# microsoft/ORBIT-Dataset

Hardware: AMD Instinct MI355X
Metric: query frames/sec per task (224×224, 5-way ProtoNet) + frame accuracy vs ref (higher is better)
Workload: dtype f32

## Files before the change

include/orbit_hip.h:

```cpp
#ifndef ORBIT_HIP_H
#define ORBIT_HIP_H

#include <stddef.h>
#include <stdint.h>

#ifdef __cplusplus
extern "C" {
#endif

typedef struct orbit_extractor orbit_extractor_t;
typedef struct orbit_filmgen orbit_filmgen_t;
typedef struct orbit_vit orbit_vit_t;
typedef void* orbit_stream_t;

#define ORBIT_OK 0
#define ORBIT_ERR_ARG (-1)
#define ORBIT_ERR_HIP (-2)
#define ORBIT_ERR_STATE (-3)
#define ORBIT_ERR_NOMEM (-4)

#define ORBIT_ACT_NONE 0
#define ORBIT_ACT_RELU 1
#define ORBIT_ACT_SILU 2
#define ORBIT_ACT_ELU 3
// ... 22 lines not shown
                        int n_tasks, int M, int T, int D, int C, float logit_scale, int cosine,
                        float* logits, int32_t* argmax, orbit_stream_t stream);

int orbit_mean_pool(const float* x, int N, int T, int D, float* out, orbit_stream_t stream);

int orbit_history_mean_pool(const float* x, int F, int T, int D, float* out, orbit_stream_t stream);
int orbit_set_mean(const float* x, int n, int D, float* out, orbit_stream_t stream);

int orbit_extractor_create(const char* name, int H, int W, orbit_extractor_t** out);
#define ORBIT_PLAN_UNFUSED 1
int orbit_extractor_create_ex(const char* name, int H, int W, int flags, orbit_extractor_t** out);
void orbit_extractor_destroy(orbit_extractor_t* fe);

int orbit_extractor_num_params(const orbit_extractor_t* fe);
const char* orbit_extractor_param_name(const orbit_extractor_t* fe, int i);
size_t orbit_extractor_param_numel(const orbit_extractor_t* fe, int i);

int orbit_extractor_load(orbit_extractor_t* fe, const char* key, const float* data, size_t numel);
int orbit_extractor_load_async(orbit_extractor_t* fe, const char* key, const float* device_data, size_t numel,
                               orbit_stream_t stream);
int orbit_extractor_load_all_async(orbit_extractor_t* fe, const float* const* device_ptrs, int n, orbit_stream_t stream);
int orbit_extractor_finalize(orbit_extractor_t* fe, orbit_stream_t stream);

int orbit_extractor_output_size(const orbit_extractor_t* fe);
int orbit_extractor_film_slots(const orbit_extractor_t* fe);
int orbit_extractor_film_slot_channels(const orbit_extractor_t* fe, int slot);
const char* orbit_extractor_film_slot_name(const orbit_extractor_t* fe, int slot);
int orbit_extractor_film_size(const orbit_extractor_t* fe);

size_t orbit_extractor_workspace_bytes(const orbit_extractor_t* fe, int B);
double orbit_extractor_macs_per_frame(const orbit_extractor_t* fe);

int orbit_extractor_forward(orbit_extractor_t* fe, const float* frames, int B,
                            const float* film_gamma, const float* film_beta,
                            float* feats, void* workspace, size_t workspace_bytes, orbit_stream_t stream);

int orbit_vit_create(const char* name, int H, int W, orbit_vit_t** out);
void orbit_vit_destroy(orbit_vit_t* v);
int orbit_vit_num_params(const orbit_vit_t* v);
const char* orbit_vit_param_name(const orbit_vit_t* v, int i);
size_t orbit_vit_param_numel(const orbit_vit_t* v, int i);
int orbit_vit_load(orbit_vit_t* v, const char* key, const float* data, size_t numel);
int orbit_vit_load_async(orbit_vit_t* v, const char* key, const float* device_data, size_t numel, orbit_stream_t stream);
int orbit_vit_load_all_async(orbit_vit_t* v, const float* const* device_ptrs, int n, orbit_stream_t stream);
int orbit_vit_finalize(orbit_vit_t* v, orbit_stream_t stream);
int orbit_vit_output_size(const orbit_vit_t* v);
int orbit_vit_film_slots(const orbit_vit_t* v);
int orbit_vit_film_slot_channels(const orbit_vit_t* v, int slot);
const char* orbit_vit_film_slot_name(const orbit_vit_t* v, int slot);
int orbit_vit_film_size(const orbit_vit_t* v);
size_t orbit_vit_workspace_bytes(const orbit_vit_t* v, int B);
double orbit_vit_macs_per_frame(const orbit_vit_t* v);
int orbit_vit_forward(orbit_vit_t* v, const float* frames, int B, const float* film_gamma, const float* film_beta,
                      float* feats, void* workspace, size_t workspace_bytes, orbit_stream_t stream);
size_t orbit_vit_tape_bytes(const orbit_vit_t* v, int B);
size_t orbit_vit_backward_workspace_bytes(const orbit_vit_t* v, int B);
int orbit_vit_train_forward(orbit_vit_t* v, const float* frames, int B, const float* film_gamma, const float* film_beta,
                            float* feats, void* tape, size_t tape_bytes, void* workspace, size_t workspace_bytes,
                            orbit_stream_t stream);
int orbit_vit_backward(orbit_vit_t* v, int B, const float* film_gamma, const float* film_beta, const float* dfeats,
                       const void* tape, size_t tape_bytes, float* dgamma, float* dbeta, void* workspace,
                       size_t workspace_bytes, orbit_stream_t stream);

int orbit_filmgen_create(int n_gen, int z_dim, int hidden, const int* out_size, const int* kind,
                         const int* dst_offset, orbit_filmgen_t** out);
void orbit_filmgen_destroy(orbit_filmgen_t* g);
int orbit_filmgen_load(orbit_filmgen_t* g, int gen, const char* tensor, const float* data, size_t numel);
int orbit_filmgen_load_all_async(orbit_filmgen_t* g, const float* const* device_ptrs, int n, orbit_stream_t stream);
int orbit_filmgen_forward(orbit_filmgen_t* g, const float* z, float* film_gamma, float* film_beta,
                          float* l2, orbit_stream_t stream);

int orbit_op_conv2d(const float* x, int x_nchw, const float* w, float* y,
                    const float* scale, const float* shift, const float* residual, const float* gate,
                    int B, int H, int W, int Cin, int Cout, int KH, int KW, int stride,
                    int pad_top, int pad_left, int Ho, int Wo, int act, int pool2,
                    orbit_stream_t stream);
int orbit_op_pw_stream(const float* x, const float* w, const float* scale, const float* shift, const float* residual,
                       const float* partial, int chunks, const float* w1, const float* b1, const float* w2t, const float* b2,
                       int R, float* y, float* gate_out, int B, int H, int W, int Cin, int Cout, orbit_stream_t stream);
int orbit_pw_stream_supported(int Cin, int Cout, int H, int W);
int orbit_op_dwconv2d(const float* x, const float* w, float* y, const float* scale, const float* shift,
                      int B, int H, int W, int C, int K, int stride, int pad_top, int pad_left,
                      int Ho, int Wo, int act, orbit_stream_t stream);
int orbit_op_conv2d_train(const float* x, int x_nchw, const float* w, float* y, const float* gate, int B, int H, int W,
                          int Cin, int Cout, int KH, int KW, int stride, int pad_top, int pad_left, int Ho, int Wo,
                          float* stats, int* stat_blocks, orbit_stream_t stream);
int orbit_op_dwconv2d_train(const float* x, const float* w, float* y, const float* in_scale, const float* in_shift,
                            int in_act, int B, int H, int W, int C, int K, int stride, int pad_top, int pad_left, int Ho,
                            int Wo, float* stats, orbit_stream_t stream);
int orbit_op_maxpool2d(const float* x, float* y, int B, int H, int W, int C, int K, int stride, int pad,
                       int Ho, int Wo, orbit_stream_t stream);
int orbit_op_avgpool(const float* x, float* y, int B, int HW, int C, orbit_stream_t stream);
int orbit_op_se_gate(const float* pooled, const float* w1, const float* b1, const float* w2,
                     const float* b2, float* gate, int B, int C, int R, orbit_stream_t stream);

int orbit_op_vit_linear(const float* x, const float* w, const float* bias, const float* residual, float* y, int M, int N,
                        int K, int epilogue, int tile_rows, orbit_stream_t stream);
int orbit_op_vit_patch_embed(const float* frames, const float* w, const float* bias_or_null, const float* pos_embed,
                             const float* cls_token, float* tokens, int B, int D, int tile_rows, orbit_stream_t stream);
int orbit_op_vit_layernorm(const float* x, size_t x_stride, float* y, size_t y_stride, int rows, int D, const float* gamma,
                           const float* beta, float eps, orbit_stream_t stream);
int orbit_op_vit_attention(const float* qkv, float* out, int B, int D, int heads, orbit_stream_t stream);
int orbit_op_vit_linear_dgrad(const float* dy, const float* w, float* wt_scratch, const float* u, const float* residual,
                              float* dx, int M, int N, int K, int tile_rows, orbit_stream_t stream);
int orbit_op_vit_layernorm_bwd(const float* x, size_t x_stride, const float* dy, size_t dy_stride, const float* gamma, float eps,
                               const float* dres, float* dx, size_t dx_stride, int rows, int D, float* dgamma, float* dbeta,
                               float* partial, size_t partial_floats, orbit_stream_t stream);
int orbit_op_vit_attention_bwd(const float* qkv, const float* dout, float* dqkv, int B, int D, int heads,
                               orbit_stream_t stream);

int orbit_op_mbconv_front_partials(int H, int W, int Cin, int mid, int K, int stride);
int orbit_op_mbconv_front(const float* x, const float* w1, const float* scale1, const float* shift1,
                          const float* wdw, const float* scale2, const float* shift2, float* y, float* pool_partial,
                          int B, int H, int W, int Cin, int mid, int K, int stride, int pad_top, int pad_left,
                          int Ho, int Wo, orbit_stream_t stream);
int orbit_op_stem_dw_front_partials(int H, int W, int mid);
int orbit_op_stem_dw_front(const float* frames, const float* w_stem, const float* scale1, const float* shift1,
                           const float* wdw, const float* scale2, const float* shift2, float* y, float* pool_partial,
                           int B, int FH, int FW, int spad_top, int spad_left, int H, int W, int mid, int pad_top,
                           int pad_left, int Ho, int Wo, orbit_stream_t stream);

int orbit_dense_rows(const float* x, int R, int in, const float* W, const float* b, int out, int act,
                     const float* residual, float* y, orbit_stream_t stream);
int orbit_spd_inverse(const float* A, float* Ainv, int n, int batch, orbit_stream_t stream);
size_t orbit_mahalanobis_workspace_bytes(int N, int M, int D, int C);
int orbit_mahalanobis_configure(const float* features, const int64_t* labels, const int64_t* class_ids, int N, int D,
                                int C, float* means, float* task_mean, float* precisions, float* task_precision,
                                void* workspace, size_t workspace_bytes, orbit_stream_t stream);
int orbit_mahalanobis_predict(const float* features, const float* means, const float* precisions, int M, int D, int C,
                              float logit_scale, float* logits, void* workspace, size_t workspace_bytes,
                              orbit_stream_t stream);

int orbit_mahalanobis_predict_backward(const float* dlogits, const float* features, const float* means,
                                       const float* precisions, int M, int D, int C, float logit_scale, float* dfeatures,
                                       void* workspace, size_t workspace_bytes, orbit_stream_t stream);

int orbit_extractor_supports_training(const orbit_extractor_t* fe);
size_t orbit_extractor_tape_bytes(const orbit_extractor_t* fe, int B);
size_t orbit_extractor_backward_workspace_bytes(const orbit_extractor_t* fe, int B);
size_t orbit_extractor_grad_floats(const orbit_extractor_t* fe);
size_t orbit_extractor_param_offset(const orbit_extractor_t* fe, int i);
size_t orbit_extractor_bn_stat_floats(const orbit_extractor_t* fe);
int orbit_extractor_export_bn_stats(orbit_extractor_t* fe, float* dst, orbit_stream_t stream);
int orbit_extractor_train_forward(orbit_extractor_t* fe, const float* frames, int B, const float* film_gamma,
                                  const float* film_beta, int bn_train, float momentum, float* feats, void* tape,
                                  size_t tape_bytes, orbit_stream_t stream);
#define ORBIT_TRAIN_NO_BACKWARD 1
#define ORBIT_TRAIN_DEFER_RUNNING_STATS 2
int orbit_extractor_train_forward_ex(orbit_extractor_t* fe, const float* frames, int B, const float* film_gamma,
                                     const float* film_beta, int bn_train, float momentum, float* feats, void* tape,
                                     size_t tape_bytes, int flags, orbit_stream_t stream);
int orbit_extractor_apply_deferred_bn_stats(orbit_extractor_t* fe, const void* tape, size_t tape_bytes, int B, float momentum,
                                            orbit_stream_t stream);
int orbit_extractor_backward(orbit_extractor_t* fe, const float* frames, int B, const float* film_gamma,
                             const float* film_beta, int bn_train, const float* dfeats, const void* tape,
                             size_t tape_bytes, float* param_grads, int filter_grads, float* dfilm_gamma,
                             float* dfilm_beta, void* workspace, size_t workspace_bytes, orbit_stream_t stream);
int orbit_extractor_train_graph_stats(const orbit_extractor_t* fe, long* replays, long* eager);
size_t orbit_filmgen_grad_floats(const orbit_filmgen_t* g);
size_t orbit_filmgen_param_offset(const orbit_filmgen_t* g, int gen, const char* tensor);
int orbit_filmgen_backward(orbit_filmgen_t* g, const float* z, const float* dfilm_gamma, const float* dfilm_beta,
                           const float* dl2, float* grads, float* dz, orbit_stream_t stream);
int orbit_proto_predict_backward(const float* dlogits, const float* features, const float* weight, int M, int T, int D,
                                 int C, float logit_scale, int cosine, float* dfeatures, orbit_stream_t stream);

int orbit_linear_head_backward(const float* dlogits, const float* features, int M, int D, int C, float logit_scale,
// ... 77 lines not shown
```

orbit-dataset_amd/_lib.py:

```python
import ctypes
import os
from ctypes import c_char_p, c_double, c_float, c_int, c_size_t, c_void_p, POINTER

_HERE = os.path.dirname(os.path.abspath(__file__))
LIB_PATH = os.path.join(_HERE, "lib", "liborbit_hip.so")

_lib = None

P = c_void_p
_SIGNATURES = {
    "orbit_version": (c_int, []),
    "orbit_last_error": (c_char_p, []),
    "orbit_device_count": (c_int, []),
    "orbit_set_option": (c_int, [c_char_p, c_int]),
    "orbit_get_option": (c_int, [c_char_p]),
    "orbit_label_set": (c_int, [P, c_int, P, c_int, P, P]),
    "orbit_proto_configure": (c_int, [P, P, P, c_int, c_int, c_int, c_int, c_int, P, P, P]),
    "orbit_proto_finalize": (c_int, [P, P, c_int, c_int, c_int, c_int, P, P, P]),
    "orbit_proto_predict": (c_int, [P, P, P, c_int, c_int, c_int, c_int, c_int, c_float, c_int, P, P, P]),
    "orbit_mean_pool": (c_int, [P, c_int, c_int, c_int, P, P]),
    "orbit_set_mean": (c_int, [P, c_int, c_int, P, P]),
    "orbit_history_mean_pool": (c_int, [P, c_int, c_int, c_int, P, P]),
    "orbit_extractor_create": (c_int, [c_char_p, c_int, c_int, POINTER(c_void_p)]),
    "orbit_extractor_create_ex": (c_int, [c_char_p, c_int, c_int, c_int, POINTER(c_void_p)]),
    "orbit_extractor_destroy": (None, [P]),
    "orbit_extractor_num_params": (c_int, [P]),
    "orbit_extractor_param_name": (c_char_p, [P, c_int]),
    "orbit_extractor_param_numel": (c_size_t, [P, c_int]),
    "orbit_extractor_load": (c_int, [P, c_char_p, P, c_size_t]),
    "orbit_extractor_load_async": (c_int, [P, c_char_p, P, c_size_t, P]),
    "orbit_extractor_load_all_async": (c_int, [P, P, c_int, P]),
    "orbit_extractor_finalize": (c_int, [P, P]),
    "orbit_extractor_output_size": (c_int, [P]),
    "orbit_extractor_film_slots": (c_int, [P]),
    "orbit_extractor_film_slot_channels": (c_int, [P, c_int]),
    "orbit_extractor_film_slot_name": (c_char_p, [P, c_int]),
    "orbit_extractor_film_size": (c_int, [P]),
    "orbit_extractor_workspace_bytes": (c_size_t, [P, c_int]),
    "orbit_extractor_macs_per_frame": (c_double, [P]),
    "orbit_extractor_forward": (c_int, [P, P, c_int, P, P, P, P, c_size_t, P]),
    "orbit_vit_create": (c_int, [c_char_p, c_int, c_int, POINTER(c_void_p)]),
    "orbit_vit_destroy": (None, [P]),
    "orbit_vit_num_params": (c_int, [P]),
    "orbit_vit_param_name": (c_char_p, [P, c_int]),
    "orbit_vit_param_numel": (c_size_t, [P, c_int]),
    "orbit_vit_load": (c_int, [P, c_char_p, P, c_size_t]),
    "orbit_vit_load_async": (c_int, [P, c_char_p, P, c_size_t, P]),
    "orbit_vit_load_all_async": (c_int, [P, P, c_int, P]),
    "orbit_vit_finalize": (c_int, [P, P]),
    "orbit_vit_output_size": (c_int, [P]),
    "orbit_vit_film_slots": (c_int, [P]),
    "orbit_vit_film_slot_channels": (c_int, [P, c_int]),
    "orbit_vit_film_slot_name": (c_char_p, [P, c_int]),
    "orbit_vit_film_size": (c_int, [P]),
    "orbit_vit_workspace_bytes": (c_size_t, [P, c_int]),
    "orbit_vit_macs_per_frame": (c_double, [P]),
    "orbit_vit_forward": (c_int, [P, P, c_int, P, P, P, P, c_size_t, P]),
    "orbit_vit_tape_bytes": (c_size_t, [P, c_int]),
    "orbit_vit_backward_workspace_bytes": (c_size_t, [P, c_int]),
    "orbit_vit_train_forward": (c_int, [P, P, c_int, P, P, P, P, c_size_t, P, c_size_t, P]),
    "orbit_vit_backward": (c_int, [P, c_int, P, P, P, P, c_size_t, P, P, P, c_size_t, P]),
    "orbit_filmgen_create": (c_int, [c_int, c_int, c_int, POINTER(c_int), POINTER(c_int), POINTER(c_int),
                                     POINTER(c_void_p)]),
    "orbit_filmgen_destroy": (None, [P]),
    "orbit_filmgen_load": (c_int, [P, c_int, c_char_p, P, c_size_t]),
    "orbit_filmgen_load_all_async": (c_int, [P, P, c_int, P]),
    "orbit_filmgen_forward": (c_int, [P, P, P, P, P, P]),
    "orbit_op_conv2d": (c_int, [P, c_int, P, P, P, P, P, P] + [c_int] * 14 + [P]),
    "orbit_op_dwconv2d": (c_int, [P, P, P, P, P] + [c_int] * 11 + [P]),
    "orbit_op_pw_stream": (c_int, [P] * 6 + [c_int] + [P] * 4 + [c_int, P, P] + [c_int] * 5 + [P]),
    "orbit_pw_stream_supported": (c_int, [c_int] * 4),
    "orbit_op_conv2d_train": (c_int, [P, c_int, P, P, P] + [c_int] * 12 + [P, POINTER(c_int), P]),
    "orbit_op_dwconv2d_train": (c_int, [P, P, P, P, P] + [c_int] * 11 + [P, P]),
    "orbit_op_maxpool2d": (c_int, [P, P] + [c_int] * 9 + [P]),
    "orbit_op_avgpool": (c_int, [P, P, c_int, c_int, c_int, P]),
    "orbit_op_se_gate": (c_int, [P, P, P, P, P, P, c_int, c_int, c_int, P]),
    "orbit_op_vit_linear": (c_int, [P] * 5 + [c_int] * 5 + [P]),
    "orbit_op_vit_patch_embed": (c_int, [P] * 6 + [c_int] * 3 + [P]),
    "orbit_op_vit_layernorm": (c_int, [P, c_size_t, P, c_size_t, c_int, c_int, P, P, c_float, P]),
    "orbit_op_vit_attention": (c_int, [P, P, c_int, c_int, c_int, P]),
    "orbit_op_vit_linear_dgrad": (c_int, [P] * 6 + [c_int] * 4 + [P]),
    "orbit_op_vit_layernorm_bwd": (c_int, [P, c_size_t, P, c_size_t, P, c_float, P, P, c_size_t, c_int, c_int, P, P, P,
                                           c_size_t, P]),
    "orbit_op_vit_attention_bwd": (c_int, [P, P, P, c_int, c_int, c_int, P]),
    "orbit_op_mbconv_front": (c_int, [P] * 9 + [c_int] * 11 + [P]),
    "orbit_op_mbconv_front_partials": (c_int, [c_int] * 6),
    "orbit_op_stem_dw_front_partials": (c_int, [c_int] * 3),
    "orbit_op_stem_dw_front": (c_int, [P] * 9 + [c_int] * 12 + [P]),
    "orbit_dense_rows": (c_int, [P, c_int, c_int, P, P, c_int, c_int, P, P, P]),
    "orbit_spd_inverse": (c_int, [P, P, c_int, c_int, P]),
    "orbit_mahalanobis_workspace_bytes": (c_size_t, [c_int, c_int, c_int, c_int]),
    "orbit_mahalanobis_configure": (c_int, [P, P, P, c_int, c_int, c_int, P, P, P, P, P, c_size_t, P]),
    "orbit_mahalanobis_predict": (c_int, [P, P, P, c_int, c_int, c_int, c_float, P, P, c_size_t, P]),
    "orbit_mahalanobis_predict_backward": (c_int, [P, P, P, P, c_int, c_int, c_int, c_float, P, P, c_size_t, P]),
    "orbit_extractor_supports_training": (c_int, [P]),
    "orbit_extractor_tape_bytes": (c_size_t, [P, c_int]),
    "orbit_extractor_backward_workspace_bytes": (c_size_t, [P, c_int]),
    "orbit_extractor_grad_floats": (c_size_t, [P]),
    "orbit_extractor_param_offset": (c_size_t, [P, c_int]),
    "orbit_extractor_bn_stat_floats": (c_size_t, [P]),
    "orbit_extractor_export_bn_stats": (c_int, [P, P, P]),
    "orbit_extractor_train_forward": (c_int, [P, P, c_int, P, P, c_int, c_float, P, P, c_size_t, P]),
    "orbit_extractor_train_forward_ex": (c_int, [P, P, c_int, P, P, c_int, c_float, P, P, c_size_t, c_int, P]),
    "orbit_extractor_apply_deferred_bn_stats": (c_int, [P, P, c_size_t, c_int, c_float, P]),
    "orbit_extractor_backward": (c_int, [P, P, c_int, P, P, c_int, P, P, c_size_t, P, c_int, P, P, P, c_size_t, P]),
    "orbit_filmgen_grad_floats": (c_size_t, [P]),
    "orbit_filmgen_param_offset": (c_size_t, [P, c_int, c_char_p]),
    "orbit_filmgen_backward": (c_int, [P, P, P, P, P, P, P, P]),
    "orbit_proto_predict_backward": (c_int, [P, P, P, c_int, c_int, c_int, c_int, c_float, c_int, P, P]),
    "orbit_linear_head_backward": (c_int, [P, P, c_int, c_int, c_int, c_float, P, P, P]),
    "orbit_cross_entropy_forward": (c_int, [P, P, c_int, c_int, c_int, P, P, P, P]),
    "orbit_cross_entropy_backward": (c_int, [P, P, P, c_int, c_int, c_int, P, P]),
    "orbit_op_bn_train_forward": (c_int, [P, c_int, c_int, P, P, c_float, c_float, P, P, P, c_int, P, P, P, P]),
    "orbit_op_bn_stats_from_gram": (c_int, [P, c_int, c_int, P, c_int, c_float, P, P, P]),
    "orbit_op_bn_backward": (c_int, [P, P, P, c_int, c_int, P, P, P, c_int, c_int, P, P, P, P, P]),
    "orbit_op_conv2d_dgrad": (c_int, [P, P, P, P] + [c_int] * 12 + [P]),
    "orbit_op_conv2d_wgrad": (c_int, [P, c_int, P, P] + [c_int] * 12 + [P]),
    "orbit_op_conv2d_wgrad_gated": (c_int, [P, P, P, P] + [c_int] * 5 + [P]),
    "orbit_op_maxpool2d_train": (c_int, [P, P, P] + [c_int] * 9 + [P]),
    "orbit_op_maxpool2d_backward": (c_int, [P, P, P] + [c_int] * 9 + [P]),
    "orbit_op_avgpool_backward": (c_int, [P, P, c_int, c_int, c_int, P]),
    "orbit_op_dwconv2d_backward": (c_int, [P, P, P, P, P] + [c_int] * 10 + [P]),
    "orbit_op_dwconv2d_dgrad_bn": (c_int, [P] * 7 + [c_int, P, P, P] + [c_int] * 10 + [P]),
    "orbit_op_dwconv2d_wgrad_xf": (c_int, [P, P, P, c_int, P, P] + [c_int] * 10 + [P]),
    "orbit_op_se_gate_backward": (c_int, [P] * 12 + [c_int] * 4 + [P]),
    "orbit_frames_from_uint8": (c_int, [P, c_int, c_int, c_int, c_int, POINTER(c_float), POINTER(c_float), P, P]),
    "orbit_prof_enable": (c_int, [c_int]),
    "orbit_prof_collect": (c_int, [POINTER(c_double), POINTER(c_double), POINTER(ctypes.c_long)]),
    "orbit_prof_num_variants": (c_int, []),
    "orbit_prof_variant": (c_int, [c_int, ctypes.c_char_p, POINTER(ctypes.c_long), POINTER(c_double),
                                   POINTER(c_double), POINTER(c_double)]),
    "orbit_prof_set_roofs": (c_int, [c_double, c_double, c_double]),
    "orbit_prof_variant_floor": (c_int, [c_int, POINTER(c_double), POINTER(c_double), POINTER(c_double)]),
    "orbit_runtime_init": (c_int, []),
    "orbit_comm_unique_id": (c_int, [P]),
    "orbit_comm_init": (c_int, [c_int, c_int, P]),
    "orbit_comm_world": (c_int, []),
    "orbit_comm_rank": (c_int, []),
    "orbit_allreduce_sum": (c_int, [P, c_size_t, P]),
    "orbit_extractor_train_graph_stats": (c_int, [P, P, P]),
    "orbit_comm_destroy": (None, []),
    "orbit_p2p_create": (c_int, [c_int, c_int, c_size_t, POINTER(c_void_p)]),
    "orbit_p2p_export": (c_int, [P, P]),
    "orbit_p2p_connect": (c_int, [P, P]),
    "orbit_p2p_allreduce_sum": (c_int, [P, P, c_size_t, P]),
    "orbit_p2p_allreduce_sum_sharded": (c_int, [P, P, c_size_t, P]),
    "orbit_p2p_error": (c_int, [P]),
    "orbit_p2p_memory_kind": (c_int, [P]),
    "orbit_p2p_destroy": (None, [P]),
}

EXPORTS = tuple(_SIGNATURES)
# ... 120 lines not shown
```

orbit-dataset_amd/csrc/ops.hip:

```cpp
#include "common.h"
#include "device_util.h"
#include "se_gate.h"
#include <algorithm>

namespace orbit {

using v4f = __attribute__((ext_vector_type(4))) float;

struct DwInXf {
    const float* scale;
    const float* shift;
    int act;
};
struct DwBnbVec {
    v4f sc, sh, mu, is;
};
__device__ __forceinline__ v4f dw_bnb(v4f dx, v4f yv, const DwBnbVec& b, int act, v4f& s0, v4f& s1) {
    const v4f z = yv * b.sc + b.sh;
    v4f g = dx;
    if (act == ORBIT_ACT_SILU) {
#pragma unroll
        for (int k = 0; k < 4; ++k) {
            const float sg = __builtin_amdgcn_rcpf(1.0f + __expf(-z[k]));
            g[k] *= sg * (1.0f + z[k] * (1.0f - sg));
// ... 484 lines not shown
#pragma unroll
    for (int u = 0; u < 2; ++u)
        if (tid + u * 256 < K * K * cs4) wl[tid + u * 256] = wq[u];
    __syncthreads();
    v4f sc = {1.f, 1.f, 1.f, 1.f}, sh = {0.f, 0.f, 0.f, 0.f}, psum = {0.f, 0.f, 0.f, 0.f}, psq = {0.f, 0.f, 0.f, 0.f};
    if (scale) sc = *reinterpret_cast<const v4f*>(scale + c);
    if (shift) sh = *reinterpret_cast<const v4f*>(shift + c);
    const int RL = P / G;
    const int g = p % G, rl = p / G;
    float* yb = y + (size_t)b * Ho * Wo * C + c;
    DwBnbVec bv;
    const float* byb = nullptr;
    if (BNB) {
        bv.sc = *reinterpret_cast<const v4f*>(bnb.bn.scale + c), bv.sh = *reinterpret_cast<const v4f*>(bnb.bn.shift + c);
        bv.mu = *reinterpret_cast<const v4f*>(bnb.bn.mean + c), bv.is = *reinterpret_cast<const v4f*>(bnb.bn.invstd + c);
        byb = bnb.y + (size_t)b * Ho * Wo * C + c;
    }
    if (rl < RL) {
        for (int ro = rl; ro < TH; ro += RL) {
            v4f acc[4];
#pragma unroll
            for (int j = 0; j < 4; ++j) acc[j] = (v4f){0.f, 0.f, 0.f, 0.f};
            const float* t0 = tile + ((size_t)(ro * S) * IWA + g * 4 * S) * CSP + lc * 4;
            const v4f* wk = wl + lc;
            const int ho = ho0 + ro;
            v4f yv[4];
            if (BNB) {
#pragma unroll
                for (int j = 0; j < 4; ++j)
                    yv[j] = *reinterpret_cast<const v4f*>(byb + ((size_t)ho * Wo + min(g * 4 + j, Wo - 1)) * C);
            }
#pragma unroll 1
            for (int kh = 0; kh < K; ++kh) {
                v4f col[NCOL];
#pragma unroll
                for (int q = 0; q < NCOL; ++q) col[q] = *reinterpret_cast<const v4f*>(t0 + q * CSP);
#pragma unroll
                for (int kw = 0; kw < K; ++kw) {
                    const v4f f = wk[kw * cs4];
#pragma unroll
                    for (int j = 0; j < 4; ++j) acc[j] += col[j * S + kw] * f;
                }
                t0 += IWA * CSP;
                wk += K * cs4;
            }
#pragma unroll
            for (int j = 0; j < 4; ++j) {
                const int wo = g * 4 + j;
                if (wo < Wo) {
                    if (BNB) {
                        *reinterpret_cast<v4f*>(yb + ((size_t)ho * Wo + wo) * C) = dw_bnb(acc[j], yv[j], bv, bnb.act, psum, psq);
                    } else {
                        v4f o = acc[j] * sc + sh;
                        o[0] = apply_act(o[0], act), o[1] = apply_act(o[1], act), o[2] = apply_act(o[2], act), o[3] = apply_act(o[3], act);
                        *reinterpret_cast<v4f*>(yb + ((size_t)ho * Wo + wo) * C) = o;
                        psum += o;
                        if (STATS) psq += o * o;
                    }
                }
            }
        }
    }
    if (pool_partial == nullptr) return;
    red[p * cs4 + lc] = psum;
    __syncthreads();
    const size_t prow = ((size_t)b * gridDim.y + chunk) * (STATS ? 2 : 1);
    if (tid < cs4) {
        v4f t = red[tid];
        for (int l = 1; l < P; ++l) t += red[l * cs4 + tid];
        *reinterpret_cast<v4f*>(pool_partial + prow * C + c0 + tid * 4) = t;
    }
    if (STATS) {
        __syncthreads();
        red[p * cs4 + lc] = psq;
        __syncthreads();
        if (tid < cs4) {
            v4f t = red[tid];
            for (int l = 1; l < P; ++l) t += red[l * cs4 + tid];
            *reinterpret_cast<v4f*>(pool_partial + (prow + 1) * C + c0 + tid * 4) = t;
        }
    }
}

template <int NT>
__global__ __launch_bounds__(NT) void se_gate2_kernel(const float* __restrict__ partial, int chunks, float inv_hw,
                                                       const float* __restrict__ w1, const float* __restrict__ b1,
                                                       const float* __restrict__ w2t, const float* __restrict__ b2,
                                                       float* __restrict__ gate, int C, int R,
                                                       float* __restrict__ pooled_out) {
    extern __shared__ __attribute__((aligned(16))) float sm2[];
    const int b = blockIdx.x;
    se_gate_frame<NT, 4>(partial + (size_t)b * chunks * C, chunks, inv_hw, w1, b1, w2t, b2, gate + (size_t)b * C, C, R,
                         pooled_out ? pooled_out + (size_t)b * C : nullptr, sm2);
}

__global__ __launch_bounds__(256) void transpose_kernel(const float* __restrict__ in, float* __restrict__ out, int rows,
                                                        int cols) {
    const int total = rows * cols;
    for (int i = blockIdx.x * 256 + threadIdx.x; i < total; i += gridDim.x * 256) {
        const int r = i / cols, c = i % cols;
        out[(size_t)c * rows + r] = in[i];
    }
}

__global__ __launch_bounds__(256) void maxpool_kernel(const float* __restrict__ x, float* __restrict__ y,
                                                      int B, int H, int W, int C, int K, int stride, int pad,
                                                      int Ho, int Wo) {
    const int C4 = C >> 2;
    const size_t total = (size_t)B * Ho * Wo * C4;
    for (size_t i = (size_t)blockIdx.x * 256 + threadIdx.x; i < total; i += (size_t)gridDim.x * 256) {
        const unsigned iu = (unsigned)i, r1 = iu / (unsigned)C4, r2 = r1 / (unsigned)Wo, bu = r2 / (unsigned)Ho;
        const int c = (int)(iu - r1 * C4) * 4, wo = (int)(r1 - r2 * Wo), ho = (int)(r2 - bu * Ho), b = (int)bu;
        const float* xb = x + (size_t)b * H * W * C + c;
        float4 m = make_float4(-INFINITY, -INFINITY, -INFINITY, -INFINITY);
        for (int kh = 0; kh < K; ++kh) {
            const int hi = ho * stride - pad + kh;
            if ((unsigned)hi >= (unsigned)H) continue;
            for (int kw = 0; kw < K; ++kw) {
                const int wi = wo * stride - pad + kw;
                if ((unsigned)wi >= (unsigned)W) continue;
                const float4 v = *reinterpret_cast<const float4*>(xb + ((size_t)hi * W + wi) * C);
                m.x = fmaxf(m.x, v.x), m.y = fmaxf(m.y, v.y), m.z = fmaxf(m.z, v.z), m.w = fmaxf(m.w, v.w);
            }
        }
        *reinterpret_cast<float4*>(y + (((size_t)b * Ho + ho) * Wo + wo) * C + c) = m;
    }
}

__global__ __launch_bounds__(256) void avgpool_kernel(const float* __restrict__ x, float* __restrict__ y,
                                                      int HW, int C) {
    __shared__ float part[4][64];
    const int b = blockIdx.y;
    const int cl = threadIdx.x & 63, slice = threadIdx.x >> 6;
    const int c = blockIdx.x * 64 + cl;
    float s = 0.f;
    if (c < C) {
        const float* p = x + (size_t)b * HW * C + c;
        for (int i = slice; i < HW; i += 4) s += p[(size_t)i * C];
    }
    part[slice][cl] = s;
    __syncthreads();
    if (slice == 0 && c < C)
        y[(size_t)b * C + c] = (part[0][cl] + part[1][cl] + part[2][cl] + part[3][cl]) / (float)HW;
}

__global__ __launch_bounds__(256) void se_gate_kernel(const float* __restrict__ pooled,
                                                      const float* __restrict__ w1, const float* __restrict__ b1,
                                                      const float* __restrict__ w2, const float* __restrict__ b2,
                                                      float* __restrict__ gate, int C, int R) {
    extern __shared__ float sm[];
    float* sp = sm;
    float* hid = sm + C;
    const int b = blockIdx.x;
    for (int c = threadIdx.x; c < C; c += 256) sp[c] = pooled[(size_t)b * C + c];
    __syncthreads();
    const int wave = threadIdx.x >> 6, lane = threadIdx.x & 63;
    for (int r = wave; r < R; r += 4) {
        float s = 0.f;
        for (int c = lane; c < C; c += 64) s = fmaf(w1[(size_t)r * C + c], sp[c], s);
        s = wave_sum_xor(s);
        if (lane == 0) {
            s += b1[r];
            hid[r] = s / (1.0f + expf(-s));
        }
    }
    __syncthreads();
    for (int c = threadIdx.x; c < C; c += 256) {
        float s = b2[c];
        for (int r = 0; r < R; ++r) s = fmaf(w2[(size_t)c * R + r], hid[r], s);
        gate[(size_t)b * C + c] = 1.0f / (1.0f + expf(-s));
    }
}

static int grid_for(size_t total) {
    size_t b = (total + 255) / 256;
    return (int)(b > 8192 ? 8192 : (b == 0 ? 1 : b));
}

static int dw_cb4(int C) {
    const int c4 = C / 4;
    for (int d = c4 < 64 ? c4 : 64; d >= 1; --d)
        if (c4 % d == 0) return d;
    return 1;
}
static int dwconv_se_rows_per_chunk(int Ho) { return Ho >= 56 ? 8 : (Ho >= 14 ? 7 : Ho); }
int dwconv_se_chunks(int Ho) { return cdiv(Ho, dwconv_se_rows_per_chunk(Ho)); }

DwForm dw_form_rule(int K, int stride, int Ho, bool train_form, bool lds_fits) {
    const int lds_opt = get_option("dw_lds");
    if (lds_fits && (lds_opt == 2 || (lds_opt == 1 && ((stride == 1 && (K == 5 || Ho <= 14)) || (train_form && stride == 2 && Ho < 14)))))
        return DW_LDS;
    const int win_opt = get_option("dw_window");
    if (win_opt == 2 || (win_opt == 1 && K == 3 && stride == 1 && Ho >= 14)) return DW_WINDOW;
    const int pipe_opt = get_option("dw_pipe");
    if (pipe_opt == 2 || (pipe_opt == 1 && stride == 2 && Ho >= (train_form ? 14 : 28))) return DW_PIPE;
    return DW_STREAM;
}

bool dwconv_se_window_form(int K, int stride, int Ho) { return dw_form_rule(K, stride, Ho, false) == DW_WINDOW; }

struct DwPlan {
    DwForm form;
    int cb4, rpc;
    dim3 grid;
    size_t lds;
    int cs4, G, IWA;
    bool deep;
};
static DwPlan dw_plan(int B, int C, int K, int stride, int Ho, int Wo, bool train_form) {
    DwPlan p{};
    p.cb4 = dw_cb4(C), p.rpc = dwconv_se_rows_per_chunk(Ho);
    p.form = dw_form_rule(K, stride, Ho, train_form);
    if (p.form == DW_LDS) {
        const int c4 = C / 4;
        p.G = cdiv(Wo, 4);
        for (int cand : {16, 8, 4}) {
            if (c4 % cand != 0 || p.G > 256 / cand) continue;
            p.cs4 = cand;
            if (2 * ((256 / cand) / p.G) >= p.rpc) break;
        }
        p.IWA = (4 * p.G - 1) * stride + K;
        const int IHmax = (p.rpc - 1) * stride + K;
        p.lds = ((size_t)IHmax * p.IWA * (p.cs4 * 4 + 4)) * sizeof(float) + (size_t)(K * K * p.cs4 + 256) * sizeof(float4);
        if (p.cs4 != 0 && p.lds <= 64 * 1024) {
            p.grid = dim3(c4 / p.cs4, cdiv(Ho, p.rpc), B);
            p.deep = IHmax * p.IWA > 8 * (256 / p.cs4);
            return p;
        }
        p.form = dw_form_rule(K, stride, Ho, train_form, false);
    }
    p.grid = dim3(C / 4 / p.cb4, cdiv(Ho, p.rpc), B);
    p.lds = (size_t)(K * K * p.cb4 + (256 / p.cb4) * p.cb4) * sizeof(float4);
    return p;
}

static int launch_dwconv_se_impl(const float* x, const float* w_khwc, float* y, const float* scale, const float* shift,
                                 float* pool_partial, int B, int H, int W, int C, int K, int stride, int pad_t, int pad_l, int Ho,
                                 int Wo, int act, hipStream_t s, int stats, const float* in_scale, const float* in_shift, int in_act,
                                 const DwBnBwd* bnb);

int launch_dwconv_se(const float* x, const float* w_khwc, float* y, const float* scale, const float* shift,
                     float* pool_partial, int B, int H, int W, int C, int K, int stride, int pad_t, int pad_l, int Ho,
                     int Wo, int act, hipStream_t s, int stats, const float* in_scale, const float* in_shift, int in_act, const DwBnBwd* bnb) {
    int rec = -1;
    if (conv_prof_enabled()) {
        char name[48];
        snprintf(name, sizeof(name), "dwconv<%dx%d/%d>%s", K, K, stride, bnb ? ",dgrad" : stats ? ",train" : "");
        const double out = (double)B * Ho * Wo * C;
        rec = prof_start(name, 2.0 * out * K * K, 4.0 * ((double)B * H * W * C + out * (bnb ? 2.0 : 1.0) + (double)K * K * C), s,
                         act == ORBIT_ACT_SILU ? out : 0.0);
    }
    const int rc = launch_dwconv_se_impl(x, w_khwc, y, scale, shift, pool_partial, B, H, W, C, K, stride, pad_t, pad_l, Ho, Wo, act,
                                         s, stats, in_scale, in_shift, in_act, bnb);
    prof_stop(rec, s);
    return rc;
}

static int launch_dwconv_se_impl(const float* x, const float* w_khwc, float* y, const float* scale, const float* shift,
                                 float* pool_partial, int B, int H, int W, int C, int K, int stride, int pad_t, int pad_l, int Ho,
                                 int Wo, int act, hipStream_t s, int stats, const float* in_scale, const float* in_shift, int in_act,
                                 const DwBnBwd* bnb) {
    ORBIT_REQUIRE(x && w_khwc && y, "dwconv_se: null pointer");
    if (bnb) {
        ORBIT_REQUIRE(bnb->y && bnb->bn.mean && bnb->bn.invstd && bnb->bn.scale && bnb->bn.shift && bnb->partial && bnb->nblk,
                      "dwconv_se: incomplete BatchNorm-backward epilogue");
        ORBIT_REQUIRE(!stats && !in_scale && !scale && !shift && !pool_partial && stride == 1 && act == ORBIT_ACT_NONE,
                      "dwconv_se: the BatchNorm-backward epilogue belongs to the plain stride-1 data-gradient use");
        *bnb->nblk = 0;
    }
    ORBIT_REQUIRE(!stats || pool_partial, "dwconv_se: statistics requested without a buffer");
    ORBIT_REQUIRE((in_scale == nullptr) == (in_shift == nullptr), "dwconv_se: the input transform needs scale and shift");
    ORBIT_REQUIRE(!in_scale || stats, "dwconv_se: the input transform is instantiated for the statistics form only");
    const DwInXf xf{in_scale, in_shift, in_act};
    const bool use_xf = in_scale != nullptr;
    ORBIT_REQUIRE(C % 4 == 0, "dwconv_se: C %% 4 != 0 (C=%d)", C);
    ORBIT_REQUIRE((K == 3 || K == 5) && (stride == 1 || stride == 2), "dwconv_se: K=%d stride=%d not instantiated", K,
                  stride);
    const DwPlan p = dw_plan(B, C, K, stride, Ho, Wo, stats != 0);
    const dim3 grid = p.grid;
    const size_t lds = p.lds;
    const int cb4 = p.cb4, rpc = p.rpc, cs4 = p.cs4, G = p.G, IWA = p.IWA;
    const DwInXf no_xf{nullptr, nullptr, 0};
    dw_dispatch_ks(K, stride, [&](auto kc, auto sc) {
        constexpr int KK = decltype(kc)::value, SS = decltype(sc)::value;
        switch (p.form) {
        case DW_LDS:
            if (bnb) {
                if constexpr (SS == 1)
                    dwconv_lds_kernel<KK, SS, 8, true, false, true><<<grid, 256, lds, s>>>(
                        x, w_khwc, y, nullptr, nullptr, bnb->partial, H, W, C, pad_t, pad_l, Ho, Wo, act, cs4, rpc, G, IWA, no_xf, *bnb);
                *bnb->nblk = (int)(grid.y * grid.z);
            } else if (use_xf)
                dwconv_lds_kernel<KK, SS, 8, true, true><<<grid, 256, lds, s>>>(x, w_khwc, y, scale, shift, pool_partial, H, W, C, pad_t,
                                                                               pad_l, Ho, Wo, act, cs4, rpc, G, IWA, xf);
            else if (stats)
                dwconv_lds_kernel<KK, SS, 8, true><<<grid, 256, lds, s>>>(x, w_khwc, y, scale, shift, pool_partial, H, W, C, pad_t, pad_l,
                                                                         Ho, Wo, act, cs4, rpc, G, IWA);
            else if (p.deep)
                dwconv_lds_kernel<KK, SS, 12><<<grid, 256, lds, s>>>(x, w_khwc, y, scale, shift, pool_partial, H, W, C, pad_t, pad_l, Ho,
                                                                    Wo, act, cs4, rpc, G, IWA);
            else
                dwconv_lds_kernel<KK, SS, 8><<<grid, 256, lds, s>>>(x, w_khwc, y, scale, shift, pool_partial, H, W, C, pad_t, pad_l, Ho,
                                                                   Wo, act, cs4, rpc, G, IWA);
            break;
        case DW_WINDOW: {
            constexpr int NO = KK == 3 ? 4 : (SS == 1 ? 2 : 1);
            if (bnb && bnb->wgrad_partial) {
                const size_t lds_wg = (size_t)(K * K * cb4 + 8 * 256) * sizeof(float4);
                if constexpr (SS == 1)
                    dwconv_win_kernel<KK, SS, NO, true, false, true, true><<<grid, 256, lds_wg, s>>>(
                        x, w_khwc, y, nullptr, nullptr, bnb->partial, H, W, C, pad_t, pad_l, Ho, Wo, act, cb4, rpc, no_xf, *bnb);
                *bnb->nblk = *bnb->wgrad_rows = (int)(grid.y * grid.z);
            } else if (bnb) {
                if constexpr (SS == 1)
                    dwconv_win_kernel<KK, SS, NO, true, false, true><<<grid, 256, lds, s>>>(
                        x, w_khwc, y, nullptr, nullptr, bnb->partial, H, W, C, pad_t, pad_l, Ho, Wo, act, cb4, rpc, no_xf, *bnb);
                *bnb->nblk = (int)(grid.y * grid.z);
            } else if (use_xf)
                dwconv_win_kernel<KK, SS, NO, true, true><<<grid, 256, lds, s>>>(x, w_khwc, y, scale, shift, pool_partial, H, W, C, pad_t,
                                                                                 pad_l, Ho, Wo, act, cb4, rpc, xf);
            else if (stats)
                dwconv_win_kernel<KK, SS, NO, true><<<grid, 256, lds, s>>>(x, w_khwc, y, scale, shift, pool_partial, H, W, C, pad_t, pad_l,
                                                                           Ho, Wo, act, cb4, rpc);
            else
                dwconv_win_kernel<KK, SS, NO><<<grid, 256, lds, s>>>(x, w_khwc, y, scale, shift, pool_partial, H, W, C, pad_t, pad_l, Ho,
                                                                     Wo, act, cb4, rpc);
            break;
        }
        case DW_PIPE:
            if (use_xf)
                dwconv_pipe_kernel<KK, SS, true, true><<<grid, 256, lds, s>>>(x, w_khwc, y, scale, shift, pool_partial, H, W, C, pad_t,
                                                                              pad_l, Ho, Wo, act, cb4, rpc, xf);
            else if (stats)
                dwconv_pipe_kernel<KK, SS, true><<<grid, 256, lds, s>>>(x, w_khwc, y, scale, shift, pool_partial, H, W, C, pad_t, pad_l, Ho,
                                                                        Wo, act, cb4, rpc);
            else
                dwconv_pipe_kernel<KK, SS><<<grid, 256, lds, s>>>(x, w_khwc, y, scale, shift, pool_partial, H, W, C, pad_t, pad_l, Ho, Wo,
                                                                  act, cb4, rpc);
            break;
        case DW_STREAM:
            if (use_xf)
                dwconv_se_kernel<KK, SS, true, true><<<grid, 256, lds, s>>>(x, w_khwc, y, scale, shift, pool_partial, H, W, C, pad_t, pad_l,
                                                                            Ho, Wo, act, cb4, rpc, xf);
            else if (stats)
                dwconv_se_kernel<KK, SS, true><<<grid, 256, lds, s>>>(x, w_khwc, y, scale, shift, pool_partial, H, W, C, pad_t, pad_l, Ho,
                                                                      Wo, act, cb4, rpc);
            else
                dwconv_se_kernel<KK, SS><<<grid, 256, lds, s>>>(x, w_khwc, y, scale, shift, pool_partial, H, W, C, pad_t, pad_l, Ho, Wo, act,
                                                                cb4, rpc);
            break;
        }
    });
    ORBIT_LAUNCH_CHECK();
    return ORBIT_OK;
}

int launch_se_gate2(const float* partial, int chunks, int HW, const float* w1, const float* b1, const float* w2t,
                    const float* b2, float* gate, int B, int C, int R, hipStream_t s, float* pooled_out) {
    ORBIT_REQUIRE(partial && w1 && b1 && w2t && b2 && gate, "se_gate2: null pointer");
    ORBIT_REQUIRE(C % 4 == 0, "se_gate2: C %% 4 != 0 (C=%d)", C);
    const size_t lds = (size_t)(((C + R + 3) & ~3) + 4 * 1024) * sizeof(float);
    const int rec = prof_start("se_gate", 4.0 * B * C * R, 4.0 * ((double)B * chunks * C + 2.0 * C * R + C + R + (double)B * C), s);
    if (C >= 1024)
        se_gate2_kernel<1024><<<B, 1024, lds, s>>>(partial, chunks, 1.0f / (float)HW, w1, b1, w2t, b2, gate, C, R, pooled_out);
    else
        se_gate2_kernel<256><<<B, 256, lds, s>>>(partial, chunks, 1.0f / (float)HW, w1, b1, w2t, b2, gate, C, R, pooled_out);
    prof_stop(rec, s);
    ORBIT_LAUNCH_CHECK();
    return ORBIT_OK;
}

int launch_transpose(const float* in, float* out, int rows, int cols, hipStream_t s) {
    transpose_kernel<<<grid_for((size_t)rows * cols), 256, 0, s>>>(in, out, rows, cols);
    ORBIT_LAUNCH_CHECK();
    return ORBIT_OK;
}

int dwconv_pack_weights(const float* w, float* w_khwc, int C, int K, hipStream_t s) {
    dw_pack_kernel<<<grid_for((size_t)C * K * K), 256, 0, s>>>(w, w_khwc, C, K);
    ORBIT_LAUNCH_CHECK();
    return ORBIT_OK;
}

int launch_maxpool(const float* x, float* y, int B, int H, int W, int C, int K, int stride, int pad, int Ho,
                   int Wo, hipStream_t s) {
    ORBIT_REQUIRE(x && y, "maxpool: null pointer");
    ORBIT_REQUIRE(C % 4 == 0, "maxpool: C %% 4 != 0 (C=%d)", C);
    const size_t total = (size_t)B * Ho * Wo * (C / 4);
    ORBIT_REQUIRE(total < (1ull << 32), "maxpool: tensor too large for 32-bit index arithmetic");
    const int rec = prof_start("maxpool", 0.0, 4.0 * ((double)B * H * W * C + (double)B * Ho * Wo * C), s);
    maxpool_kernel<<<grid_for(total), 256, 0, s>>>(x, y, B, H, W, C, K, stride, pad, Ho, Wo);
    prof_stop(rec, s);
    ORBIT_LAUNCH_CHECK();
    return ORBIT_OK;
}

int launch_avgpool(const float* x, float* y, int B, int HW, int C, hipStream_t s) {
    ORBIT_REQUIRE(x && y && B > 0 && HW > 0 && C > 0, "avgpool: bad arguments");
    dim3 grid(cdiv(C, 64), B);
    const int rec = prof_start("avgpool", (double)B * HW * C, 4.0 * ((double)B * HW * C + (double)B * C), s);
    avgpool_kernel<<<grid, 256, 0, s>>>(x, y, HW, C);
    prof_stop(rec, s);
    ORBIT_LAUNCH_CHECK();
    return ORBIT_OK;
}

int launch_se_gate(const float* pooled, const float* w1, const float* b1, const float* w2, const float* b2,
                   float* gate, int B, int C, int R, hipStream_t s) {
    ORBIT_REQUIRE(pooled && w1 && b1 && w2 && b2 && gate, "se_gate: null pointer");
    se_gate_kernel<<<B, 256, (size_t)(C + R) * sizeof(float), s>>>(pooled, w1, b1, w2, b2, gate, C, R);
    ORBIT_LAUNCH_CHECK();
    return ORBIT_OK;
}

}

using namespace orbit;

extern "C" {

int orbit_op_dwconv2d(const float* x, const float* w, float* y, const float* scale, const float* shift, int B,
                      int H, int W, int C, int K, int stride, int pad_top, int pad_left, int Ho, int Wo,
                      int act, orbit_stream_t stream) {
    ORBIT_REQUIRE(x && w && y, "op_dwconv2d: null pointer");
    hipStream_t s = (hipStream_t)stream;
    float* wp = nullptr;
    ORBIT_HIP_CHECK(hipMallocAsync(reinterpret_cast<void**>(&wp), (size_t)C * K * K * sizeof(float), s));
    int rc = dwconv_pack_weights(w, wp, C, K, s);
    if (rc == ORBIT_OK)
        rc = launch_dwconv_se(x, wp, y, scale, shift, nullptr, B, H, W, C, K, stride, pad_top, pad_left, Ho, Wo, act, s);
    (void)hipFreeAsync(wp, s);
    return rc;
}

int orbit_op_dwconv2d_train(const float* x, const float* w, float* y, const float* in_scale, const float* in_shift,
                            int in_act, int B, int H, int W, int C, int K, int stride, int pad_top, int pad_left, int Ho,
                            int Wo, float* stats, orbit_stream_t stream) {
    ORBIT_REQUIRE(x && w && y && stats, "op_dwconv2d_train: null pointer");
    hipStream_t s = (hipStream_t)stream;
    const int nblk = B * dwconv_se_chunks(Ho);
    float* tmp = nullptr;
    const size_t wfl = (size_t)C * K * K, pfl = bn_partial_floats((size_t)nblk, C) + 4 * (size_t)C;
    ORBIT_HIP_CHECK(hipMallocAsync(reinterpret_cast<void**>(&tmp), (wfl + pfl) * sizeof(float), s));
    float* part = tmp + ((wfl + 63) & ~(size_t)63);
    int rc = dwconv_pack_weights(w, tmp, C, K, s);
    if (rc == ORBIT_OK)
        rc = launch_dwconv_se(x, tmp, y, nullptr, nullptr, part, B, H, W, C, K, stride, pad_top, pad_left, Ho, Wo,
                              ORBIT_ACT_NONE, s, 1, in_scale, in_shift, in_act);
    if (rc == ORBIT_OK) rc = launch_sum_partials(part, nblk, C, stats, s);
    (void)hipFreeAsync(tmp, s);
    return rc;
}

int orbit_op_maxpool2d(const float* x, float* y, int B, int H, int W, int C, int K, int stride, int pad,
                       int Ho, int Wo, orbit_stream_t stream) {
    return launch_maxpool(x, y, B, H, W, C, K, stride, pad, Ho, Wo, (hipStream_t)stream);
}

int orbit_op_avgpool(const float* x, float* y, int B, int HW, int C, orbit_stream_t stream) {
    return launch_avgpool(x, y, B, HW, C, (hipStream_t)stream);
}

int orbit_op_se_gate(const float* pooled, const float* w1, const float* b1, const float* w2, const float* b2,
                     float* gate, int B, int C, int R, orbit_stream_t stream) {
    return launch_se_gate(pooled, w1, b1, w2, b2, gate, B, C, R, (hipStream_t)stream);
}

}
```

Baseline: 38240.

## Add multi-frame LDS depthwise conv kernel with prefetch for small 5x5 layers

Adds a depthwise-conv kernel variant in which each block processes several frames in sequence. It keeps the packed weights in LDS and loads the next frame's input tile into registers while computing the current one. Inference-only 5x5 stride-1 layers with output height up to 7 use it, two frames per block by default. The intent is to amortise weight staging and launch overhead on tiny late-stage layers at the cost of fewer blocks and extra synchronisation. A pooled-output variant of the op API is also exposed.

```diff
diff --git a/include/orbit_hip.h b/include/orbit_hip.h
--- a/include/orbit_hip.h
+++ b/include/orbit_hip.h
@@ -128,6 +128,10 @@
 int orbit_op_dwconv2d(const float* x, const float* w, float* y, const float* scale, const float* shift,
                       int B, int H, int W, int C, int K, int stride, int pad_top, int pad_left,
                       int Ho, int Wo, int act, orbit_stream_t stream);
+int orbit_op_dwconv2d_pool(const float* x, const float* w, float* y, const float* scale, const float* shift,
+                           float* pool_partial, int B, int H, int W, int C, int K, int stride, int pad_top, int pad_left,
+                           int Ho, int Wo, int act, orbit_stream_t stream);
+int orbit_op_dwconv2d_pool_chunks(int Ho);
 int orbit_op_conv2d_train(const float* x, int x_nchw, const float* w, float* y, const float* gate, int B, int H, int W,
                           int Cin, int Cout, int KH, int KW, int stride, int pad_top, int pad_left, int Ho, int Wo,
                           float* stats, int* stat_blocks, orbit_stream_t stream);
diff --git a/orbit-dataset_amd/_lib.py b/orbit-dataset_amd/_lib.py
--- a/orbit-dataset_amd/_lib.py
+++ b/orbit-dataset_amd/_lib.py
@@ -68,6 +68,8 @@
     "orbit_filmgen_forward": (c_int, [P, P, P, P, P, P]),
     "orbit_op_conv2d": (c_int, [P, c_int, P, P, P, P, P, P] + [c_int] * 14 + [P]),
     "orbit_op_dwconv2d": (c_int, [P, P, P, P, P] + [c_int] * 11 + [P]),
+    "orbit_op_dwconv2d_pool": (c_int, [P, P, P, P, P, P] + [c_int] * 11 + [P]),
+    "orbit_op_dwconv2d_pool_chunks": (c_int, [c_int]),
     "orbit_op_pw_stream": (c_int, [P] * 6 + [c_int] + [P] * 4 + [c_int, P, P] + [c_int] * 5 + [P]),
     "orbit_pw_stream_supported": (c_int, [c_int] * 4),
     "orbit_op_conv2d_train": (c_int, [P, c_int, P, P, P] + [c_int] * 12 + [P, POINTER(c_int), P]),
diff --git a/orbit-dataset_amd/csrc/ops.hip b/orbit-dataset_amd/csrc/ops.hip
--- a/orbit-dataset_amd/csrc/ops.hip
+++ b/orbit-dataset_amd/csrc/ops.hip
@@ -590,6 +590,158 @@
     }
 }
 
+template <int K, int CS4, int U>
+__global__ __launch_bounds__(256, K == 5 ? (U > 8 ? 3 : 4) : 4) void dwconv_lds_frames_kernel(
+    const float* __restrict__ x, const float* __restrict__ w, float* __restrict__ y, const float* __restrict__ scale,
+    const float* __restrict__ shift, float* __restrict__ pool_partial, int B, int H, int W, int C, int pad_t, int pad_l, int Ho,
+    int Wo, int act, int rows_per_chunk, int G, int IWA, int F) {
+    constexpr int NCOL = 3 + K;
+    constexpr int CSP = CS4 * 4 + 4;
+    constexpr int P = 256 / CS4;
+    constexpr unsigned NONE = ~0u;
+    extern __shared__ __attribute__((aligned(16))) float smf[];
+    const int chunk = blockIdx.y;
+    const int b0 = blockIdx.z * F, nf = min(F, B - b0);
+    const int c0 = blockIdx.x * CS4 * 4;
+    const int ho0 = chunk * rows_per_chunk;
+    const int TH = min(Ho, ho0 + rows_per_chunk) - ho0;
+    const int IH = TH - 1 + K;
+    const int IHmax = rows_per_chunk - 1 + K;
+    float* tile = smf;
+    v4f* wl = reinterpret_cast<v4f*>(smf + (size_t)IHmax * IWA * CSP);
+    v4f* red = wl + K * K * CS4;
+    const int tid = threadIdx.x;
+    const int lc = tid % CS4, p = tid / CS4;
+    const int c = c0 + lc * 4;
+    v4f wq[2] = {{0.f, 0.f, 0.f, 0.f}, {0.f, 0.f, 0.f, 0.f}};
+#pragma unroll
+    for (int u = 0; u < 2; ++u) {
+        const int i = tid + u * 256;
+        if (i < K * K * CS4) wq[u] = *reinterpret_cast<const v4f*>(w + (size_t)(i / CS4) * C + c0 + (i % CS4) * 4);
+    }
+    const int hi0 = ho0 - pad_t;
+    const int n_items = IH * IWA;
+    const int dr = P / IWA, dc = P % IWA;
+    const size_t xfs = (size_t)H * W * C, yfs = (size_t)Ho * Wo * C;
+    unsigned src[U];
+    {
+        int r = p / IWA, col = p % IWA;
+#pragma unroll
+        for (int u = 0; u < U; ++u) {
+            const int hi = hi0 + r, wi = col - pad_l;
+            src[u] = (p + u * P < n_items && (unsigned)hi < (unsigned)H && (unsigned)wi < (unsigned)W) ? (unsigned)((hi * W + wi) * C + c) : NONE;
+            r += dr, col += dc;
+            if (col >= IWA) col -= IWA, ++r;
+        }
+    }
+    float* tp = tile + p * CSP + lc * 4;
+    auto stage_rest = [&](const float* xf) {
+        const int first = p + U * P;
+        int r = first / IWA, col = first % IWA;
+        for (int i0 = first; i0 < n_items; i0 += 8 * P) {
+            v4f v[8];
+            int dst[8];
+#pragma unroll
+            for (int u = 0; u < 8; ++u) {
+                const bool in = i0 + u * P < n_items;
+                const int hi = hi0 + r, wi = col - pad_l;
+                v[u] = (v4f){0.f, 0.f, 0.f, 0.f};
+                dst[u] = in ? (r * IWA + col) * CSP + lc * 4 : -1;
+                if (in && (unsigned)hi < (unsigned)H && (unsigned)wi < (unsigned)W)
+                    v[u] = *reinterpret_cast<const v4f*>(xf + (unsigned)((hi * W + wi) * C + c));
+                r += dr, col += dc;
+                if (col >= IWA) col -= IWA, ++r;
+            }
+#pragma unroll
+            for (int u = 0; u < 8; ++u)
+                if (dst[u] >= 0) *reinterpret_cast<v4f*>(tile + dst[u]) = v[u];
+        }
+    };
+    const float* xf = x + (size_t)b0 * xfs;
+    float* yf = y + (size_t)b0 * yfs;
+    {
+        v4f v[U];
+#pragma unroll
+        for (int u = 0; u < U; ++u) {
+            v[u] = (v4f){0.f, 0.f, 0.f, 0.f};
+            if (src[u] != NONE) v[u] = *reinterpret_cast<const v4f*>(xf + src[u]);
+        }
+#pragma unroll
+        for (int u = 0; u < U; ++u)
+            if (p + u * P < n_items) *reinterpret_cast<v4f*>(tp + u * P * CSP) = v[u];
+        if (n_items > U * P) stage_rest(xf);
+    }
+#pragma unroll
+    for (int u = 0; u < 2; ++u)
+        if (tid + u * 256 < K * K * CS4) wl[tid + u * 256] = wq[u];
+    __syncthreads();
+    v4f sc = {1.f, 1.f, 1.f, 1.f}, sh = {0.f, 0.f, 0.f, 0.f};
+    if (scale) sc = *reinterpret_cast<const v4f*>(scale + c);
+    if (shift) sh = *reinterpret_cast<const v4f*>(shift + c);
+    const int RL = P / G;
+    const int g = p % G, rl = p / G;
+    for (int f = 0; f < nf; ++f, xf += xfs, yf += yfs) {
+        const bool more = f + 1 < nf;
+        v4f v[U];
+#pragma unroll
+        for (int u = 0; u < U; ++u) {
+            v[u] = (v4f){0.f, 0.f, 0.f, 0.f};
+            if (more && src[u] != NONE) v[u] = *reinterpret_cast<const v4f*>(xf + xfs + src[u]);
+        }
+        v4f psum = {0.f, 0.f, 0.f, 0.f};
+        if (rl < RL) {
+            for (int ro = rl; ro < TH; ro += RL) {
+                v4f acc[4];
+#pragma unroll
+                for (int j = 0; j < 4; ++j) acc[j] = (v4f){0.f, 0.f, 0.f, 0.f};
+                const float* t0 = tile + (ro * IWA + g * 4) * CSP + lc * 4;
+                const v4f* wk = wl + lc;
+                const int ho = ho0 + ro;
+#pragma unroll 1
+                for (int kh = 0; kh < K; ++kh) {
+                    v4f col[NCOL];
+#pragma unroll
+                    for (int q = 0; q < NCOL; ++q) col[q] = *reinterpret_cast<const v4f*>(t0 + q * CSP);
+#pragma unroll
+                    for (int kw = 0; kw < K; ++kw) {
+                        const v4f fw = wk[kw * CS4];
+#pragma unroll
+                        for (int j = 0; j < 4; ++j) acc[j] += col[j + kw] * fw;
+                    }
+                    t0 += IWA * CSP;
+                    wk += K * CS4;
+                }
+#pragma unroll
+                for (int j = 0; j < 4; ++j) {
+                    const int wo = g * 4 + j;
+                    if (wo < Wo) {
+                        v4f o = acc[j] * sc + sh;
+                        o[0] = apply_act(o[0], act), o[1] = apply_act(o[1], act), o[2] = apply_act(o[2], act), o[3] = apply_act(o[3], act);
+                        *reinterpret_cast<v4f*>(yf + (unsigned)((ho * Wo + wo) * C + c)) = o;
+                        psum += o;
+                    }
+                }
+            }
+        }
+        if (pool_partial) red[p * CS4 + lc] = psum;
+        if (more || pool_partial) __syncthreads();
+        if (more) {
+#pragma unroll
+            for (int u = 0; u < U; ++u)
+                if (src[u] != NONE) *reinterpret_cast<v4f*>(tp + u * P * CSP) = v[u];
+            if (n_items > U * P) stage_rest(xf + xfs);
+        }
+        if (pool_partial && tid < CS4) {
+            const size_t prow = (size_t)(b0 + f) * gridDim.y + chunk;
+            v4f t = red[tid];
+#pragma unroll
+            for (int l = 1; l < P; ++l) t += red[l * CS4 + tid];
+            *reinterpret_cast<v4f*>(pool_partial + prow * C + c0 + tid * 4) = t;
+        }
+        if (more) __syncthreads();
+    }
+}
+
 template <int NT>
 __global__ __launch_bounds__(NT) void se_gate2_kernel(const float* __restrict__ partial, int chunks, float inv_hw,
                                                        const float* __restrict__ w1, const float* __restrict__ b1,
@@ -695,7 +847,7 @@
 int dwconv_se_chunks(int Ho) { return cdiv(Ho, dwconv_se_rows_per_chunk(Ho)); }
 
 DwForm dw_form_rule(int K, int stride, int Ho, bool train_form, bool lds_fits) {
-    const int lds_opt = get_option("dw_lds");
+    const int lds_opt = min(get_option("dw_lds"), 2);
     if (lds_fits && (lds_opt == 2 || (lds_opt == 1 && ((stride == 1 && (K == 5 || Ho <= 14)) || (train_form && stride == 2 && Ho < 14)))))
         return DW_LDS;
     const int win_opt = get_option("dw_window");
@@ -707,6 +859,12 @@
 
 bool dwconv_se_window_form(int K, int stride, int Ho) { return dw_form_rule(K, stride, Ho, false) == DW_WINDOW; }
 
+static int dw_frames_rule(int K, int stride, int Ho) {
+    const int opt = get_option("dw_lds");
+    if (opt >= 16) return min(opt - 16, 64);
+    return K == 5 && stride == 1 && Ho <= 7 ? 2 : 0;
+}
+
 struct DwPlan {
     DwForm form;
     int cb4, rpc;
@@ -714,8 +872,9 @@
     size_t lds;
     int cs4, G, IWA;
     bool deep;
+    int frames;
 };
-static DwPlan dw_plan(int B, int C, int K, int stride, int Ho, int Wo, bool train_form) {
+static DwPlan dw_plan(int B, int C, int K, int stride, int Ho, int Wo, bool train_form, bool inference) {
     DwPlan p{};
     p.cb4 = dw_cb4(C), p.rpc = dwconv_se_rows_per_chunk(Ho);
     p.form = dw_form_rule(K, stride, Ho, train_form);
@@ -731,7 +890,8 @@
         const int IHmax = (p.rpc - 1) * stride + K;
         p.lds = ((size_t)IHmax * p.IWA * (p.cs4 * 4 + 4)) * sizeof(float) + (size_t)(K * K * p.cs4 + 256) * sizeof(float4);
         if (p.cs4 != 0 && p.lds <= 64 * 1024) {
-            p.grid = dim3(c4 / p.cs4, cdiv(Ho, p.rpc), B);
+            p.frames = inference && stride == 1 ? dw_frames_rule(K, stride, Ho) : 0;
+            p.grid = dim3(c4 / p.cs4, cdiv(Ho, p.rpc), p.frames ? cdiv(B, p.frames) : B);
             p.deep = IHmax * p.IWA > 8 * (256 / p.cs4);
             return p;
         }
@@ -784,7 +944,7 @@
     ORBIT_REQUIRE(C % 4 == 0, "dwconv_se: C %% 4 != 0 (C=%d)", C);
     ORBIT_REQUIRE((K == 3 || K == 5) && (stride == 1 || stride == 2), "dwconv_se: K=%d stride=%d not instantiated", K,
                   stride);
-    const DwPlan p = dw_plan(B, C, K, stride, Ho, Wo, stats != 0);
+    const DwPlan p = dw_plan(B, C, K, stride, Ho, Wo, stats != 0, !stats && !bnb && !use_xf);
     const dim3 grid = p.grid;
     const size_t lds = p.lds;
     const int cb4 = p.cb4, rpc = p.rpc, cs4 = p.cs4, G = p.G, IWA = p.IWA;
@@ -804,6 +964,17 @@
             else if (stats)
                 dwconv_lds_kernel<KK, SS, 8, true><<<grid, 256, lds, s>>>(x, w_khwc, y, scale, shift, pool_partial, H, W, C, pad_t, pad_l,
                                                                          Ho, Wo, act, cs4, rpc, G, IWA);
+            else if (p.frames) {
+                if constexpr (SS == 1) {
+                    auto go = [&](auto csc, auto uc) {
+                        dwconv_lds_frames_kernel<KK, decltype(csc)::value, decltype(uc)::value><<<grid, 256, lds, s>>>(
+                            x, w_khwc, y, scale, shift, pool_partial, B, H, W, C, pad_t, pad_l, Ho, Wo, act, rpc, G, IWA, p.frames);
+                    };
+                    using std::integral_constant;
+                    auto go_u = [&](auto csc) { p.deep ? go(csc, integral_constant<int, 9>{}) : go(csc, integral_constant<int, 7>{}); };
+                    cs4 == 16 ? go_u(integral_constant<int, 16>{}) : cs4 == 8 ? go_u(integral_constant<int, 8>{}) : go_u(integral_constant<int, 4>{});
+                }
+            }
             else if (p.deep)
                 dwconv_lds_kernel<KK, SS, 12><<<grid, 256, lds, s>>>(x, w_khwc, y, scale, shift, pool_partial, H, W, C, pad_t, pad_l, Ho,
                                                                     Wo, act, cs4, rpc, G, IWA);
@@ -927,19 +1098,27 @@
 
 extern "C" {
 
-int orbit_op_dwconv2d(const float* x, const float* w, float* y, const float* scale, const float* shift, int B,
-                      int H, int W, int C, int K, int stride, int pad_top, int pad_left, int Ho, int Wo,
-                      int act, orbit_stream_t stream) {
+int orbit_op_dwconv2d_pool(const float* x, const float* w, float* y, const float* scale, const float* shift,
+                           float* pool_partial, int B, int H, int W, int C, int K, int stride, int pad_top, int pad_left, int Ho,
+                           int Wo, int act, orbit_stream_t stream) {
     ORBIT_REQUIRE(x && w && y, "op_dwconv2d: null pointer");
     hipStream_t s = (hipStream_t)stream;
     float* wp = nullptr;
     ORBIT_HIP_CHECK(hipMallocAsync(reinterpret_cast<void**>(&wp), (size_t)C * K * K * sizeof(float), s));
     int rc = dwconv_pack_weights(w, wp, C, K, s);
     if (rc == ORBIT_OK)
-        rc = launch_dwconv_se(x, wp, y, scale, shift, nullptr, B, H, W, C, K, stride, pad_top, pad_left, Ho, Wo, act, s);
+        rc = launch_dwconv_se(x, wp, y, scale, shift, pool_partial, B, H, W, C, K, stride, pad_top, pad_left, Ho, Wo, act, s);
     (void)hipFreeAsync(wp, s);
     return rc;
 }
+
+int orbit_op_dwconv2d(const float* x, const float* w, float* y, const float* scale, const float* shift, int B,
+                      int H, int W, int C, int K, int stride, int pad_top, int pad_left, int Ho, int Wo,
+                      int act, orbit_stream_t stream) {
+    return orbit_op_dwconv2d_pool(x, w, y, scale, shift, nullptr, B, H, W, C, K, stride, pad_top, pad_left, Ho, Wo, act, stream);
+}
+
+int orbit_op_dwconv2d_pool_chunks(int Ho) { return dwconv_se_chunks(Ho); }
 
 int orbit_op_dwconv2d_train(const float* x, const float* w, float* y, const float* in_scale, const float* in_shift,
                             int in_act, int B, int H, int W, int C, int K, int stride, int pad_top, int pad_left, int Ho,
```

New measurement: 38070. No clear change (-0.4%).
